# spiraldb/fastlanes

Measured on AMD Instinct MI355X. Metric: billion integers/sec decoded (u32 width-7) + achieved HBM GB/s vs peak, 1-8 GPU, higher is better.
Workload: dtype u32

## Files before the change

__graft_entry__.py:

```python
import os
import subprocess
import sys

ROOT = os.path.dirname(os.path.abspath(__file__))
if ROOT not in sys.path:
    sys.path.insert(0, ROOT)


def build_library():
    jobs = str(min(8, os.cpu_count() or 1))
    subprocess.check_call(["make", "-s", "-j", jobs, "-C", os.path.join(ROOT, "fastlanes_amd", "csrc")])


def build_oracle():
    subprocess.check_call(["make", "-s", "-C", os.path.join(ROOT, "oracle")])


EXAMPLES = ("fused_dict_decode", "iterate_running_max", "fused_for_pack")


def build_examples():
    deps0 = [os.path.join(ROOT, "fastlanes_amd", "csrc", h) for h in ("fl_device.hpp", "fl_kernels.hpp", "fl_tile_map.hpp")]
    outs = {}
    for name in EXAMPLES:
        src = os.path.join(ROOT, "examples", name + ".hip")
        out = os.path.join(ROOT, "examples", "lib" + name + ".so")
        deps = [src] + deps0
        if not os.path.exists(out) or any(os.path.getmtime(d) > os.path.getmtime(out) for d in deps):
            subprocess.check_call(["/opt/rocm/bin/hipcc", "--offload-arch=gfx950", "-O3", "-std=c++17", "-shared", "-fPIC",
                                   "-I", os.path.join(ROOT, "fastlanes_amd", "csrc"), src, "-o", out])
        outs[name] = out
    for name, extra in (("column_decode", []), ("multi_gpu_decode", ["-lpthread"])):
        src = os.path.join(ROOT, "examples", name + ".c")
        exe = os.path.join(ROOT, "examples", name)
        if not os.path.exists(exe) or os.path.getmtime(src) > os.path.getmtime(exe) or \
                os.path.getmtime(os.path.join(ROOT, "include", "fastlanes_amd.h")) > os.path.getmtime(exe):
            subprocess.check_call(["gcc", "-std=c99", "-O2", "-Wall", "-D__HIP_PLATFORM_AMD__", "-I", os.path.join(ROOT, "include"),
                                   "-I", "/opt/rocm/include", src, "-L", os.path.join(ROOT, "fastlanes_amd"), "-lfastlanes_amd",
                                   "-L", "/opt/rocm/lib", "-lamdhip64", "-Wl,-rpath,$ORIGIN/../fastlanes_amd",
                                   "-Wl,-rpath,/opt/rocm/lib"] + extra + ["-o", exe])
        outs[name] = exe
    return outs


def build_checker():
    sys.path.insert(0, os.path.join(ROOT, "tests"))
    from test_gpu_full_check import build_checker as bc
    return bc()


def build():
    build_library()
    build_oracle()
    build_examples()
    build_checker()
    import fastlanes_amd
    lib = fastlanes_amd.load()
    missing = [s for s in fastlanes_amd.exported_symbols() + fastlanes_amd.for_compare_symbols() + fastlanes_amd.select_symbols() +
               fastlanes_amd.aggregate_symbols() + fastlanes_amd.for_compare_range_symbols() + fastlanes_amd.aggregate_by_symbols() + fastlanes_amd.for_compare_columns_symbols() +
               fastlanes_amd.aggregate_columns_symbols() + fastlanes_amd.for_compare_in_symbols() + fastlanes_amd.aggregate_by_columns_symbols() if not hasattr(lib, s)]
    if missing:
        raise RuntimeError(f"libfastlanes_amd.so lacks {missing}")


def smoke():
    import numpy as np
    import torch

    sys.path.insert(0, os.path.join(ROOT, "tests"))
    import fastlanes_amd as fl
    from datagen import values
    from oracle_lib import load_oracle

    assert torch.cuda.is_available(), "smoke() needs cuda:0"
    fl.load()
    oracle = load_oracle()
    dev = torch.device("cuda:0")
    n = 70

    def to_dev(a):
        return torch.from_numpy(a.view(np.uint8)).to(dev).view(getattr(torch, str(a.dtype)))

    def to_np(t, dt):
        return t.view(torch.uint8).cpu().numpy().view(dt)

    pk = values("u32", n * 224, 1)
    got = to_np(fl.BitPacking.unpack(7, to_dev(pk)), np.uint32)
    assert np.array_equal(got, oracle.batch("unpack", "u32", 7, pk)), "unpack u32 W=7 mismatch"
    v = values("u32", n * 1024, 2)
    got = to_np(fl.BitPacking.pack(7, to_dev(v)), np.uint32)
    assert np.array_equal(got, oracle.batch("pack", "u32", 7, v)), "pack u32 W=7 mismatch"
    pk12 = values("u32", n * 384, 3)
    bases = values("u32", n * 32, 4)
    got = to_np(fl.Delta.undelta_pack(12, to_dev(pk12), to_dev(bases)), np.uint32)
    assert np.array_equal(got, oracle.batch("undelta_pack", "u32", 12, pk12, aux=bases)), "undelta_pack mismatch"
    refs = values("u32", n, 5)
    got = to_np(fl.FoR.unfor_pack(7, to_dev(pk), to_dev(refs)), np.uint32)
    assert np.array_equal(got, oracle.batch("unfor_pack", "u32", 7, pk, aux=refs)), "unfor_pack mismatch"
    v64 = values("u64", n * 1024, 6, bits=17)
    d = to_dev(v64)
    assert torch.equal(fl.BitPacking.unpack(17, fl.BitPacking.pack(17, d)).view(torch.int64), d.view(torch.int64))
    v16 = (np.arange(1024) % 8).astype(np.uint16)
    p16 = fl.BitPacking.pack(3, v16)
    assert np.array_equal(p16, oracle.pack("u16", 3, v16))
    assert np.array_equal(fl.BitPacking.unpack(3, p16), v16)
    widths = (1 + np.arange(n) % 32).astype(np.uint8)
    dw = torch.from_numpy(widths).to(dev)
    doff, dtotal = fl.widths_to_offsets("u32", dw)
    off = np.concatenate([[0], np.cumsum(widths.astype(np.int64) * 32)])
    assert int(dtotal.item()) == off[-1] * 4
    col = values("u32", int(off[-1]), 7)
    got = to_np(fl.unpack_widths(dw, doff, to_dev(col)), np.uint32)
    want = np.concatenate([oracle.unpack("u32", int(w), col[off[b]:off[b + 1]]) for b, w in enumerate(widths)])
    assert np.array_equal(got, want), "unpack_widths mismatch"
    brefs = values("u32", n, 8)
    got = to_np(fl.unfor_pack_widths(dw, doff, to_dev(col), to_dev(brefs)), np.uint32)
    want = np.concatenate([oracle.unfor_pack("u32", int(w), col[off[b]:off[b + 1]], brefs[b]) for b, w in enumerate(widths)])
    assert np.array_equal(got, want), "unfor_pack_widths mismatch"
    got = to_np(fl.undelta_pack_widths(dw, doff, to_dev(col), to_dev(bases)), np.uint32)
    want = np.concatenate([oracle.undelta_pack("u32", int(w), col[off[b]:off[b + 1]], bases[b * 32:(b + 1) * 32]) for b, w in enumerate(widths)])
    assert np.array_equal(got, want), "undelta_pack_widths mismatch"
    n8 = 4 * n + 3
    w8 = ((np.arange(n8) * 5) % 9).astype(np.uint8)
    dw8 = torch.from_numpy(w8).to(dev)
    doff8, _ = fl.widths_to_offsets("u8", dw8)
    off8 = np.concatenate([[0], np.cumsum(w8.astype(np.int64) * 128)])
    col8, bases8 = values("u8", int(off8[-1]), 9), values("u8", n8 * 128, 10)
    want = np.concatenate([oracle.undelta_pack("u8", int(w), col8[off8[b]:off8[b + 1]], bases8[b * 128:(b + 1) * 128]) for b, w in enumerate(w8)])
    got = to_np(fl.undelta_pack_widths(dw8, doff8, to_dev(col8), to_dev(bases8)), np.uint8)
    assert np.array_equal(got, want), "undelta_pack_widths u8 mismatch"
# ... 25 lines not shown
```

fastlanes_amd/csrc/fl_capi.hip:

```cpp
#include "../../include/fastlanes_amd.h"
#include "../../include/fastlanes_amd_internal.h"
#include "fl_host.hpp"
#include "fl_kernels.hpp"
#include "fl_misc.hpp"
#include "fl_widths.hpp"
#include "fl_chain.hpp"
#include "fl_stream.hpp"
#include "fl_batch.hpp"
#include "fl_scan.hpp"
#include "fl_consume.hpp"
#include "fl_for_compare.hpp"
#include "fl_for_compare_range.hpp"
#include "fl_for_compare_in.hpp"
#include "fl_aggregate_by_columns.hpp"
#include "fl_select.hpp"
#include "fl_aggregate.hpp"
#include "fl_aggregate_by.hpp"
#include "fl_for_compare_columns.hpp"
#include "fl_aggregate_columns.hpp"
#include "fl_host_tier.hpp"

#include <algorithm>
#include <atomic>
#include <new>
// ... 943 lines not shown
    {                                                                                                     \
        FL_DEVICE_TIER(s, aw, ao, a, ar, bw, bo, b, br, kw, ko, k, kr, mask, res, ef);                    \
        return run_unfor_aggregate_by_columns<T>(ex, {true, 0, aw, ao, ab}, a, ar, ars, {true, 0, bw, bo, bb}, b, br, brs, {true, 0, kw, ko, kb}, k, \
                                                 kr, krs, mask, n, res, ef, s);                           \
    }

FL_DEFINE_AGGREGATE_BY_COLUMNS(uint8_t, u8)
FL_DEFINE_AGGREGATE_BY_COLUMNS(uint16_t, u16)
FL_DEFINE_AGGREGATE_BY_COLUMNS(uint32_t, u32)
FL_DEFINE_AGGREGATE_BY_COLUMNS(uint64_t, u64)

#define FL_DEFINE_FOR_COMPARE_RANGE(T, S)                                                               \
    int fl_##S##_unfor_compare_range(unsigned w, const T* in, const T* r, size_t rs, T lo, T hi, int cb, const uint32_t* mi, size_t n, \
                                     uint32_t* mask, void* s)                                             \
    { FL_DEVICE_TIER(s, in, r, mi, mask); return run_unfor_compare_range<T>({false, w}, in, r, rs, lo, hi, cb, mi, n, mask, nullptr, s); } \
    int fl_##S##_unfor_compare_range_widths(const uint8_t* w, const uint64_t* o, const T* pk, size_t pb, const T* r, size_t rs, T lo, T hi, \
                                            int cb, const uint32_t* mi, size_t n, uint32_t* mask, uint32_t* ef, void* s) \
    { FL_DEVICE_TIER(s, w, o, pk, r, mi, mask, ef); return run_unfor_compare_range<T>({true, 0, w, o, pb}, pk, r, rs, lo, hi, cb, mi, n, mask, ef, s); }

FL_DEFINE_FOR_COMPARE_RANGE(uint8_t, u8)
FL_DEFINE_FOR_COMPARE_RANGE(uint16_t, u16)
FL_DEFINE_FOR_COMPARE_RANGE(uint32_t, u32)
FL_DEFINE_FOR_COMPARE_RANGE(uint64_t, u64)

#define FL_DEFINE_FOR_COMPARE_IN(T, S)                                                                    \
    int fl_##S##_unfor_compare_in(unsigned w, const T* in, const T* r, size_t rs, T lo, uint64_t sb, const uint32_t* sw, int ng, int cb, \
                                  const uint32_t* mi, size_t n, uint32_t* mask, void* s)                  \
    { FL_DEVICE_TIER(s, in, r, sw, mi, mask); return run_unfor_compare_in<T>({false, w}, in, r, rs, lo, sb, sw, ng, cb, mi, n, mask, nullptr, s); } \
    int fl_##S##_unfor_compare_in_widths(const uint8_t* w, const uint64_t* o, const T* pk, size_t pb, const T* r, size_t rs, T lo, uint64_t sb, \
                                         const uint32_t* sw, int ng, int cb, const uint32_t* mi, size_t n, uint32_t* mask, uint32_t* ef, void* s) \
    { FL_DEVICE_TIER(s, w, o, pk, r, sw, mi, mask, ef); return run_unfor_compare_in<T>({true, 0, w, o, pb}, pk, r, rs, lo, sb, sw, ng, cb, mi, n, mask, ef, s); }

FL_DEFINE_FOR_COMPARE_IN(uint8_t, u8)
FL_DEFINE_FOR_COMPARE_IN(uint16_t, u16)
FL_DEFINE_FOR_COMPARE_IN(uint32_t, u32)
FL_DEFINE_FOR_COMPARE_IN(uint64_t, u64)

#define FL_DEFINE_FOR_COMPARE_COLUMNS(T, S)                                                               \
    int fl_##S##_unfor_compare_columns(unsigned wa, const T* a, const T* ar, size_t ars, unsigned wb, const T* b, const T* br, size_t brs, \
                                       int op, int sg, int cb, const uint32_t* mi, size_t n, uint32_t* mask, void* s) \
    {                                                                                                     \
        FL_DEVICE_TIER(s, a, ar, b, br, mi, mask);                                                        \
        return run_unfor_compare_columns<T>({false, wa}, a, ar, ars, {false, wb}, b, br, brs, op, sg, cb, mi, n, mask, nullptr, s); \
    }                                                                                                     \
    int fl_##S##_unfor_compare_columns_widths(const uint8_t* aw, const uint64_t* ao, const T* a, size_t ab, const T* ar, size_t ars, \
                                              const uint8_t* bw, const uint64_t* bo, const T* b, size_t bb, const T* br, size_t brs, \
                                              int op, int sg, int cb, const uint32_t* mi, size_t n, uint32_t* mask, uint32_t* ef, void* s) \
    {                                                                                                     \
        FL_DEVICE_TIER(s, aw, ao, a, ar, bw, bo, b, br, mi, mask, ef);                                    \
        return run_unfor_compare_columns<T>({true, 0, aw, ao, ab}, a, ar, ars, {true, 0, bw, bo, bb}, b, br, brs, op, sg, cb, mi, n, mask, ef, s); \
    }

FL_DEFINE_FOR_COMPARE_COLUMNS(uint8_t, u8)
FL_DEFINE_FOR_COMPARE_COLUMNS(uint16_t, u16)
FL_DEFINE_FOR_COMPARE_COLUMNS(uint32_t, u32)
FL_DEFINE_FOR_COMPARE_COLUMNS(uint64_t, u64)

#define FL_DEFINE_AGGREGATE_COLUMNS(T, S)                                                                 \
    int fl_##S##_unfor_aggregate_columns(int ex, unsigned wa, const T* a, const T* ar, size_t ars, unsigned wb, const T* b, const T* br, \
                                         size_t brs, const uint32_t* mask, size_t n, void* aggs, uint32_t* ef, void* s) \
    {                                                                                                     \
        FL_DEVICE_TIER(s, a, ar, b, br, mask, aggs, ef);                                                  \
        return run_unfor_aggregate_columns<T>(ex, {false, wa}, a, ar, ars, {false, wb}, b, br, brs, mask, n, aggs, ef, s); \
    }                                                                                                     \
    int fl_##S##_unfor_aggregate_columns_widths(int ex, const uint8_t* aw, const uint64_t* ao, const T* a, size_t ab, const T* ar, size_t ars, \
                                                const uint8_t* bw, const uint64_t* bo, const T* b, size_t bb, const T* br, size_t brs, \
                                                const uint32_t* mask, size_t n, void* aggs, uint32_t* ef, void* s) \
    {                                                                                                     \
        FL_DEVICE_TIER(s, aw, ao, a, ar, bw, bo, b, br, mask, aggs, ef);                                  \
        return run_unfor_aggregate_columns<T>(ex, {true, 0, aw, ao, ab}, a, ar, ars, {true, 0, bw, bo, bb}, b, br, brs, mask, n, aggs, ef, s); \
    }

FL_DEFINE_AGGREGATE_COLUMNS(uint8_t, u8)
FL_DEFINE_AGGREGATE_COLUMNS(uint16_t, u16)
FL_DEFINE_AGGREGATE_COLUMNS(uint32_t, u32)
FL_DEFINE_AGGREGATE_COLUMNS(uint64_t, u64)

FL_DEFINE_TYPE(uint8_t, u8)
FL_DEFINE_TYPE(uint16_t, u16)
FL_DEFINE_TYPE(uint32_t, u32)
FL_DEFINE_TYPE(uint64_t, u64)


void fl_internal_set_kernel_policy(int policy)
{
    const KernelPolicy p = policy_fields(policy);
    const bool ok = policy >= 0 && policy < (1 << 30) && p.mode <= 2 && (p.waves == 0 || (p.waves >= 3 && p.waves <= 8)) && p.bpw <= 16
                    && (p.mode == 2 || (p.waves == 0 && p.bpw == 0)) && (p.prefetch == 0 || p.bpw >= 2) && (p.window == 0 || p.window >= 8);
    g_kernel_policy.store(ok ? policy : 0, std::memory_order_relaxed);
    fl::window_override().store(ok ? p.window : 0, std::memory_order_relaxed);
}
int fl_internal_get_kernel_policy(void) { return g_kernel_policy.load(std::memory_order_relaxed); }
uint64_t fl_internal_zero_copy_fallbacks(void) { return g_zero_copy_fallbacks.load(std::memory_order_relaxed); }

int fl_internal_bare_stream(const void* in, size_t in_unit, const void* aux, size_t aux_unit, void* out, size_t out_unit, size_t n_units,
                            int nt_loads, int waves, int window_log2_units, void* stream)
{
    if (n_units == 0) return FL_OK;
    if ((in_unit && !in) || (aux_unit && !aux) || !out) return FL_ERR_NULL;
    if (misaligned(in) || misaligned(aux) || misaligned(out)) return FL_ERR_ALIGN;
    if (in_unit > BARE_MAX_UNIT || out_unit > BARE_MAX_UNIT || aux_unit > 1024 || ((in_unit | out_unit | aux_unit) & 15u)) return FL_ERR_INDEX;
    FL_DEVICE_TIER(stream, in, aux, out);
    BareArgs a{static_cast<const char*>(in), static_cast<const char*>(aux), static_cast<char*>(out), n_units, 0,
               (unsigned)in_unit, (unsigned)aux_unit, (unsigned)out_unit, 63u};
    return hip_status(launch_bare_stream(a, nt_loads != 0, waves, window_log2_units, static_cast<hipStream_t>(stream)));
}

int fl_internal_bare_stream_shape(int op, unsigned type_bits, unsigned width, size_t* in_unit, size_t* aux_unit, size_t* out_unit,
                                  int* nt_loads, int* waves, int* window_log2_units, unsigned* blocks_per_unit)
{
    if (!valid_type_bits(type_bits)) return FL_ERR_INDEX;
    if (op < 0 || op > 3) return FL_ERR_INDEX;
    if (width > (op == 3 ? 2 * type_bits : type_bits)) return FL_ERR_WIDTH;
    if (!in_unit || !aux_unit || !out_unit || !nt_loads || !waves || !window_log2_units || !blocks_per_unit) return FL_ERR_NULL;
    const unsigned k = type_bits == 8 ? 4u : type_bits == 16 ? 2u : 1u;
    const size_t packed = (op == 3 ? 64u * width : 128u * width) * k, unpacked = 128u * type_bits * k;
    *blocks_per_unit = k;
    *in_unit = op == 1 ? unpacked : packed;
    *out_unit = op == 1 ? packed : unpacked;
    *aux_unit = op == 2 ? 128u * k : 0;
    int w = op == 3 ? mixed_waves(type_bits, false) : chosen_waves(type_bits, width, tool_op(op).wave).waves;
    if (w == 0) w = 8;
    *waves = w < 3 ? 3 : w;
    *nt_loads = op == 1 || op == 3 || width >= fl::nt_read_from(type_bits);
    *window_log2_units = window_log2_blocks(tool_op(op).window, type_bits);
    return FL_OK;
}

int fl_internal_selftune_check(int op, unsigned type_bits, unsigned width, const void* in, const void* aux, void* out, size_t n_blocks, void* stream,
                               float* table_ms, float* best_other_ms, int* best_other_policy)
{
    if (!table_ms || !best_other_ms || !best_other_policy) return FL_ERR_NULL;
    if (op < 0 || op > 2 || !valid_type_bits(type_bits)) return FL_ERR_INDEX;
    if (width > type_bits) return FL_ERR_WIDTH;
    hipStream_t s = static_cast<hipStream_t>(stream);
    auto call = [&]() -> int {
        return type_bits == 8 ? selftune_call<uint8_t>(op, width, in, aux, out, n_blocks, stream)
             : type_bits == 16 ? selftune_call<uint16_t>(op, width, in, aux, out, n_blocks, stream)
             : type_bits == 32 ? selftune_call<uint32_t>(op, width, in, aux, out, n_blocks, stream)
                               : selftune_call<uint64_t>(op, width, in, aux, out, n_blocks, stream);
    };
    const int saved = fl_internal_get_kernel_policy();
    int rc = FL_OK;
    auto timed = [&](int policy, float& ms) {
        fl_internal_set_kernel_policy(policy);
        rc = median_ms(s, 1, 3, call, &ms);
    };
    *table_ms = *best_other_ms = 0.f;
    timed(0, *table_ms);
    *best_other_policy = 0;
    const fl::WaveOp wop = tool_op(op).wave;
    const fl::WaveChoice tab = fl::wave_choice(type_bits, width, wop);
    for (int policy : {1, 2 + 256 * 3, 2 + 256 * 4, 2 + 256 * 5, 2 + 256 * 6, 2 + 256 * 8}) {
        if (rc != FL_OK) break;
        if (policy == 1 && (tab.waves == 0 || !fl::cell_column_built(type_bits, width, wop))) continue;
        if (policy != 1 && (policy >> 8) == tab.waves && !tab.two_blocks) continue;
        float ms = 0.f;
        timed(policy, ms);
        if (rc == FL_OK && ms > 0.f && (*best_other_ms == 0.f || ms < *best_other_ms)) { *best_other_ms = ms; *best_other_policy = policy; }
    }
    fl_internal_set_kernel_policy(saved);
    return rc;
}

}
```

fastlanes_amd/csrc/fl_consume.hpp:

```cpp
#pragma once
#include "fl_kernels.hpp"

namespace fl {

constexpr int compare_max_waves(int w) { return w <= 5 ? 8 : w <= 9 ? 3 : 2; }
inline int compare_launch_waves(unsigned type_bits, unsigned w) { return w > 5 ? 0 : type_bits == 8 ? 4 : type_bits == 16 ? 6 : 0; }
constexpr int sums_max_waves(int w) { return (w >= 6 && w <= 12) ? 3 : 8; }

struct ReduceArgs {
    const u32x4* in;
    void* out0;
    void* out1;
    uint64_t n_blocks;
    uint64_t tiles_per_xcd = 0;
    unsigned window_shift = 63;
};

__device__ __forceinline__ bool tile_of_workgroup(const ReduceArgs& a, uint64_t& tile)
{
    const uint64_t n_tiles = (a.n_blocks + BLOCKS_PER_WG - 1) / BLOCKS_PER_WG;
    tile = xcd_tile(blockIdx.x, a.tiles_per_xcd, a.window_shift);
    return tile < n_tiles;
}

// ... 318 lines not shown
{
    using P = InPlaceRows<T, W>;
    constexpr int TB = Elem<T>::BITS;
    auto put = [&](auto J, uint32_t bits) {
        constexpr int j = decltype(J)::value;
        static_assert(j >= 0 && j < TB, "");
        if constexpr (sizeof(T) == 1) *reinterpret_cast<uint16_t*>(lds_blk + j * 16 + c * 2) = (uint16_t)bits;
        else *reinterpret_cast<uint8_t*>(lds_blk + j * 8 + c) = (uint8_t)bits;
    };
    constexpr T FM = W >= TB ? (T) ~(T)0 : (T)(((uint32_t)1 << (W % TB)) - 1u);
    const uint32_t kc = k > FM ? FM : k;
    static_for<(W ? W : 1)>([&](auto WD) {
        constexpr int wd = decltype(WD)::value;
        static_for<2>([&](auto C) {
            constexpr int cl = decltype(C)::value;
            if constexpr (P::any(wd, cl)) {
                constexpr uint32_t M = P::fields(wd, cl), G = P::guards(wd, cl), ONES = P::ones(wd, cl);
                const uint32_t ks = kc * ONES;
                uint32_t t[4];
                for (int i = 0; i < 4; ++i) {
                    if constexpr (IS_EQ) t[i] = G - ((in[wd].x[i] ^ ks) & M);
                    else t[i] = (ks | G) - (in[wd].x[i] & M);
                }
                static_for<TB>([&](auto R) {
                    constexpr int r = decltype(R)::value;
                    static_assert(WaveRowStore<T>::row_at(P::address_row(r)) == r, "address_row inverts row_at");
                    if constexpr (P::member(r, wd, cl))
                        put(std::integral_constant<int, P::address_row(r)>{}, squeeze_bit<T, P::shift(r) + W>(t));
                });
            }
        });
    });
    static_for<TB>([&](auto R) {
        constexpr int r = decltype(R)::value;
        if constexpr (!P::in_place(r))
            put(std::integral_constant<int, P::address_row(r)>{}, row_predicate_bits<T, W, IS_EQ>(unpack_row<T, W, r>(in), (T)kc));
    });
    wave_lds_fence();
    const u32x4 m = *reinterpret_cast<const u32x4*>(lds_blk + c * 16);
    keep[0] = m[0]; keep[1] = m[1]; keep[2] = m[2]; keep[3] = m[3];
    if (IS_EQ && k > FM) keep[0] = keep[1] = keep[2] = keep[3] = 0u;
}

template <typename T, int W, bool IS_EQ>
__global__ __launch_bounds__(WG) __attribute__((amdgpu_waves_per_eu(1, compare_max_waves(W)))) void k_unpack_compare(CompareArgs a)
{
    const uint64_t n_tiles = (a.n_blocks + BLOCKS_PER_WG - 1) / BLOCKS_PER_WG;
    const uint64_t tile = xcd_tile(blockIdx.x, a.tiles_per_xcd, a.window_shift);
    if (tile >= n_tiles) return;
    const unsigned tid = threadIdx.x;
    const uint64_t blk = tile * BLOCKS_PER_WG + (tid >> 3);
    const unsigned c = sizeof(T) >= 4 ? column_of_lane(tid & 7u) : (tid & 7u);
    if (blk >= a.n_blocks) return;
    Cell<T> in[W ? W : 1];
    const u32x4* pk = a.in + blk * (uint64_t)(8 * W) + c;
    static_for<W>([&](auto Wd) { in[decltype(Wd)::value] = load_cell<T, true>(pk + 8 * decltype(Wd)::value); });
    uint32_t keep[4] = {0, 0, 0, 0};
    if constexpr (sizeof(T) >= 4) {
        compare_block_butterfly<T, W, IS_EQ>(in, (T)a.constant, c, keep);
    } else {
        constexpr unsigned MASK_STRIDE = 144;
        __shared__ __attribute__((aligned(16))) char lds[BLOCKS_PER_WG * MASK_STRIDE];
        compare_block_lds<T, W, IS_EQ>(in, (T)a.constant, c, lds + (tid >> 3) * MASK_STRIDE, keep);
    }
    const uint32_t flip = a.invert ? ~0u : 0u;
    const u32x4 out = {keep[0] ^ flip, keep[1] ^ flip, keep[2] ^ flip, keep[3] ^ flip};
    const unsigned wave = __builtin_amdgcn_readfirstlane(tid >> 6);
    const uint64_t wave_first = tile * BLOCKS_PER_WG + wave * 8u;
    const uint64_t left = a.n_blocks - wave_first;
    const __amdgpu_buffer_rsrc_t mask_rs = __builtin_amdgcn_make_buffer_rsrc(
        reinterpret_cast<char*>(a.mask) + wave_first * 128u, 0, (unsigned)(left < 8 ? left : 8) * 128u, 0x00020000);
    __builtin_amdgcn_raw_buffer_store_b128(out, mask_rs, ((tid >> 3) & 7u) * 128u + c * 16u, 0, STORE_AUX);
}

typedef hipError_t (*compare_launch_t)(const CompareArgs&, int waves, hipStream_t);
template <typename T, int W, bool IS_EQ> hipError_t launch_unpack_compare(const CompareArgs& a0, int waves, hipStream_t s)
{
    if (a0.n_blocks == 0) return hipSuccess;
    CompareArgs a = a0;
    const unsigned grid = plan_blocks(a, a.n_blocks, BLOCKS_PER_WG, WIN_UNPACK_COMPARE, Elem<T>::BITS);
    if (!grid) return hipErrorInvalidValue;
    constexpr unsigned STATIC_LDS = sizeof(T) >= 4 ? 0u : BLOCKS_PER_WG * 144u;
    unsigned pad = 0;
    if (waves >= 3 && waves < 8) pad = ((CU_LDS_BYTES / (unsigned)waves) & ~1023u) - STATIC_LDS;
    FL_LAUNCH((k_unpack_compare<T, W, IS_EQ>), dim3(grid), dim3(WG), pad, s, a);
    return hipGetLastError();
}
template <typename T> struct CompareTable { compare_launch_t fn[Elem<T>::BITS + 1]; };
template <typename T, bool IS_EQ, int... Ws>
constexpr CompareTable<T> make_compare_table(std::integer_sequence<int, Ws...>)
{
    return CompareTable<T>{{&launch_unpack_compare<T, Ws, IS_EQ>...}};
}
template <typename T, bool IS_EQ> const CompareTable<T>& compare_table_impl();

typedef hipError_t (*reduce_launch_t)(const ReduceArgs&, hipStream_t);

template <typename T, int W> hipError_t launch_unpack_block_sums(const ReduceArgs& a0, hipStream_t s)
{
    if (a0.n_blocks == 0) return hipSuccess;
    ReduceArgs a = a0;
    const unsigned grid = plan_blocks(a, a.n_blocks, BLOCKS_PER_WG, WIN_UNPACK_BLOCK_SUMS, Elem<T>::BITS);
    if (!grid) return hipErrorInvalidValue;
    FL_LAUNCH((k_unpack_block_sums<T, W>), dim3(grid), dim3(WG), 0, s, a);
    return hipGetLastError();
}
template <typename T> hipError_t launch_block_min_max(const ReduceArgs& a0, hipStream_t s)
{
    if (a0.n_blocks == 0) return hipSuccess;
    ReduceArgs a = a0;
    const unsigned grid = plan_blocks(a, a.n_blocks, BLOCKS_PER_WG, WIN_BLOCK_MIN_MAX, Elem<T>::BITS);
    if (!grid) return hipErrorInvalidValue;
    FL_LAUNCH((k_block_min_max<T>), dim3(grid), dim3(WG), 0, s, a);
    return hipGetLastError();
}

template <typename T> struct ReduceTable { reduce_launch_t fn[Elem<T>::BITS + 1]; };
template <typename T, int... Ws>
constexpr ReduceTable<T> make_sum_table(std::integer_sequence<int, Ws...>)
{
    return ReduceTable<T>{{&launch_unpack_block_sums<T, Ws>...}};
}
template <typename T> const ReduceTable<T>& sum_table_impl();
template <typename T> reduce_launch_t min_max_launcher();

}
```

fastlanes_amd/csrc/fl_dispatch.hpp:

```cpp
#pragma once
#include "fl_dispatch_table.inc"
#include "fl_window_table.inc"

namespace fl {

enum WaveOp { WAVE_UNPACK = 0, WAVE_PACK = 1, WAVE_UNDELTA_PACK = 2, WAVE_UNDELTA = 3, WAVE_DELTA = 4,
              WAVE_UNTRANSPOSE = 5, WAVE_TRANSPOSE = 6, WAVE_UNDELTA_PACK_UNTRANSPOSE = 7, WAVE_TRANSPOSE_DELTA_PACK = 8,
              WAVE_UNFOR_PACK = 9, WAVE_FOR_PACK = 10 };

#define FL_DISPATCH_ROW(NAME, type_bits) \
    ((type_bits) == 64 ? dispatch_table::NAME##_U64 : (type_bits) == 32 ? dispatch_table::NAME##_U32 : \
     (type_bits) == 16 ? dispatch_table::NAME##_U16 : dispatch_table::NAME##_U8)

constexpr int TWO_BLOCKS = 10;
namespace dispatch_table {
template <unsigned N> constexpr bool row_below(const unsigned char (&row)[N], int limit)
{
    for (unsigned i = 0; i < N; ++i)
        if (row[i] >= limit) return false;
    return true;
}
template <unsigned N> constexpr bool two_blocks_row_ok(const unsigned char (&row)[N])
{
    for (unsigned i = 0; i < N; ++i)
        if (row[i] > 8 && (row[i] < TWO_BLOCKS + 4 || row[i] > TWO_BLOCKS + 8)) return false;
    return true;
}
#define FL_CHECK_ROWS(NAME) static_assert(row_below(NAME##_U8, 9) && row_below(NAME##_U16, 9) && row_below(NAME##_U32, 9) && row_below(NAME##_U64, 9), \
                                          "fl_dispatch_table.inc: " #NAME " holds an entry that is not 0 or 3..8 waves per SIMD")
FL_CHECK_ROWS(UNPACK); FL_CHECK_ROWS(PACK); FL_CHECK_ROWS(UNFOR_PACK); FL_CHECK_ROWS(FOR_PACK); FL_CHECK_ROWS(UNDELTA_PACK_UNTRANSPOSE);
FL_CHECK_ROWS(TRANSPOSE_DELTA_PACK); FL_CHECK_ROWS(UNDELTA); FL_CHECK_ROWS(DELTA); FL_CHECK_ROWS(UNTRANSPOSE); FL_CHECK_ROWS(TRANSPOSE);
#undef FL_CHECK_ROWS
static_assert(row_below(UNDELTA_PACK_U8, 9) && row_below(UNDELTA_PACK_U16, 9), "fl_dispatch_table.inc: the two-blocks form exists for u32 / u64 only");
static_assert(two_blocks_row_ok(UNDELTA_PACK_U32) && two_blocks_row_ok(UNDELTA_PACK_U64), "fl_dispatch_table.inc: a two-blocks entry must be 10 + (4..8)");
}
constexpr int unpack_u32_floor(unsigned w, int table) { return (w >= 9 && w < 16 && table > 0 && table < 6) ? 6 : table; }
constexpr int undelta_u64_floor(unsigned w, int table) { return (w >= 8 && w <= 10 && table == 0) ? 6 : table == 3 ? 4 : table; }
constexpr int wave_policy(unsigned type_bits, unsigned w, WaveOp op)
{
    switch (op) {
    case WAVE_UNPACK: return type_bits == 32 ? unpack_u32_floor(w, dispatch_table::UNPACK_U32[w]) : FL_DISPATCH_ROW(UNPACK, type_bits)[w];
    case WAVE_PACK: return FL_DISPATCH_ROW(PACK, type_bits)[w];
    case WAVE_UNFOR_PACK: return FL_DISPATCH_ROW(UNFOR_PACK, type_bits)[w];
    case WAVE_FOR_PACK: return FL_DISPATCH_ROW(FOR_PACK, type_bits)[w];
    case WAVE_UNDELTA_PACK: return type_bits == 64 ? undelta_u64_floor(w, dispatch_table::UNDELTA_PACK_U64[w]) : FL_DISPATCH_ROW(UNDELTA_PACK, type_bits)[w];
    case WAVE_UNDELTA_PACK_UNTRANSPOSE:
        return type_bits == 64 ? undelta_u64_floor(w, dispatch_table::UNDELTA_PACK_UNTRANSPOSE_U64[w]) : FL_DISPATCH_ROW(UNDELTA_PACK_UNTRANSPOSE, type_bits)[w];
    case WAVE_TRANSPOSE_DELTA_PACK: return FL_DISPATCH_ROW(TRANSPOSE_DELTA_PACK, type_bits)[w];
    case WAVE_UNDELTA: return FL_DISPATCH_ROW(UNDELTA, type_bits)[0];
    case WAVE_DELTA: return FL_DISPATCH_ROW(DELTA, type_bits)[0];
    case WAVE_UNTRANSPOSE: return FL_DISPATCH_ROW(UNTRANSPOSE, type_bits)[0];
    default: return FL_DISPATCH_ROW(TRANSPOSE, type_bits)[0];
    }
}

struct WaveChoice {
    int waves;
    bool two_blocks;
};
constexpr WaveChoice wave_choice(unsigned type_bits, unsigned w, WaveOp op)
{
    const int e = wave_policy(type_bits, w, op);
    return e >= TWO_BLOCKS ? WaveChoice{e - TWO_BLOCKS, true} : WaveChoice{e, false};
}

#ifdef FL_ALL_CELL_COLUMN
constexpr bool cell_column_built(unsigned, unsigned, WaveOp) { return true; }
#else
constexpr bool cell_column_built(unsigned type_bits, unsigned w, WaveOp op) { return wave_policy(type_bits, w, op) == 0; }
#endif

constexpr int wave_fallback(unsigned type_bits, bool pack) { return (pack || type_bits <= 16) ? 8 : type_bits == 32 ? 5 : 3; }

inline unsigned uniform_blocks_per_wave(unsigned type_bits, bool  = false, unsigned  = 0, bool  = false)
{
    return type_bits == 8 ? 2u : 1u;
}
inline unsigned mixed_blocks_per_wave(unsigned type_bits, bool pack) { return type_bits == 8 ? (pack ? 2u : 4u) : type_bits == 16 ? 2u : 1u; }
inline unsigned nt_read_from(unsigned type_bits)
{
    static const unsigned div = [] { const char* e = getenv("FL_INTERNAL_NT_FROM_DIV"); const int d = e ? atoi(e) : 0; return d >= 1 && d <= 64 ? (unsigned)d : 0u; }();
    const unsigned d = div ? div : (type_bits >= 32 ? 8u : 2u);
    return (type_bits + d - 1) / d;
}
inline unsigned mixed_prefetch(unsigned type_bits) { return type_bits <= 16 ? 1u : 0u; }
inline int mixed_waves(unsigned type_bits, bool pack) { return (pack || type_bits <= 16) ? 8 : 6; }
inline unsigned batch_blocks_per_wave(unsigned type_bits, bool pack)
{
    return type_bits == 8 ? 4u : type_bits == 16 ? (pack ? 2u : 4u) : (type_bits == 64 && !pack) ? 2u : 1u;
}
inline int batch_waves(unsigned type_bits, bool pack) { return type_bits <= 16 ? 8 : pack ? 6 : type_bits == 64 ? 5 : 8; }

enum WindowOp { WIN_UNPACK = 0, WIN_PACK, WIN_UNDELTA_PACK, WIN_UNDELTA_PACK_UNTRANSPOSE, WIN_TRANSPOSE_DELTA_PACK, WIN_DELTA, WIN_UNDELTA,
                WIN_TRANSPOSE, WIN_UNTRANSPOSE, WIN_UNPACK_COMPARE, WIN_UNPACK_BLOCK_SUMS, WIN_BLOCK_MIN_MAX };
constexpr int window_log2_blocks(WindowOp op, unsigned type_bits)
{
    const int t = type_bits == 8 ? 0 : type_bits == 16 ? 1 : type_bits == 32 ? 2 : 3;
    switch (op) {
    case WIN_UNPACK: return window_table::UNPACK[t];
    case WIN_PACK: return window_table::PACK[t];
    case WIN_UNDELTA_PACK: return window_table::UNDELTA_PACK[t];
    case WIN_UNDELTA_PACK_UNTRANSPOSE: return window_table::UNDELTA_PACK_UNTRANSPOSE[t];
    case WIN_TRANSPOSE_DELTA_PACK: return window_table::TRANSPOSE_DELTA_PACK[t];
    case WIN_DELTA: return window_table::DELTA[t];
    case WIN_UNDELTA: return window_table::UNDELTA[t];
    case WIN_TRANSPOSE: return window_table::TRANSPOSE[t];
    case WIN_UNTRANSPOSE: return window_table::UNTRANSPOSE[t];
    case WIN_UNPACK_COMPARE: return window_table::UNPACK_COMPARE[t];
    case WIN_UNPACK_BLOCK_SUMS: return window_table::UNPACK_BLOCK_SUMS[t];
    default: return window_table::BLOCK_MIN_MAX[t];
    }
}

constexpr unsigned BATCH_MAX_BLOCKS = 1u << 30;

}
```

fastlanes_amd/csrc/fl_kernels.hpp:

```cpp
#pragma once
#include "fl_device.hpp"
#include "fl_dispatch.hpp"
#include "fl_tile_map.hpp"
#include <atomic>

namespace fl {

#ifndef FL_WG
#define FL_WG 256
#endif
constexpr int WG = FL_WG;
constexpr int BLOCKS_PER_WG = WG / 8;

enum UnpackBody { BODY_STORE = 0, BODY_ADD_REF = 1, BODY_UNDELTA = 2,
                  BODY_UNDELTA_UNTRANSPOSE = 3 };
enum PackMode { PACK_PLAIN = 0, PACK_FOR = 1,
                PACK_TRANSPOSE_DELTA = 2 };

struct StreamArgs {
    const u32x4* in;
    u32x4* out;
    const void* aux;
    uint64_t aux_stride;
    uint64_t n_blocks;
    uint64_t tiles_per_xcd = 0;
    unsigned window_shift = 63;
};


inline std::atomic<int>& window_override()
{
    static std::atomic<int> v{0};
    return v;
}
inline int& window_override_this_thread()
{
    static thread_local int v = 0;
    return v;
}
inline bool& constructed_pair_this_thread()
{
    static thread_local bool v = false;
    return v;
}
inline unsigned tile_window_shift(WindowOp op, unsigned type_bits, unsigned tile_blocks)
{
    const int mine = window_override_this_thread();
    const int ov = mine ? mine : window_override().load(std::memory_order_relaxed);
    return window_shift_of(ov ? ov : constructed_pair_this_thread() ? (int)WINDOW_WHOLE : window_log2_blocks(op, type_bits), tile_blocks);
}

template <typename Args>
inline unsigned plan_blocks(Args& a, uint64_t n_blocks, unsigned tile_blocks, WindowOp op, unsigned type_bits, bool rotate = false)
{
    return plan_tiles(a, (n_blocks + tile_blocks - 1) / tile_blocks, tile_window_shift(op, type_bits, tile_blocks) | (rotate ? TILE_MAP_ROTATE : 0u));
}
constexpr unsigned CU_LDS_BYTES = 160 * 1024;
inline unsigned occupancy_lds(int waves, unsigned need = 0)
{
    if (waves < 3) waves = 3;
    const unsigned pad = (CU_LDS_BYTES * (unsigned)WG / ((unsigned)waves * 256u)) & ~1023u;
    return pad > need ? pad : need;
}

#ifndef FL_STORE_AUX
#define FL_STORE_AUX 18
#endif
constexpr int STORE_AUX = FL_STORE_AUX;

template <typename T, int W> struct UnpackPolicy {
    static constexpr int MAXW = 2;
    static constexpr int MAXW_ROWS = 3;
    static constexpr bool NT_LOAD = (2 * W >= Elem<T>::BITS);
};
template <typename T> struct PackPolicy {
    static constexpr int MAXW = sizeof(T) >= 4 ? 1 : 2;
    static constexpr bool NT_LOAD = true;
};

__device__ __forceinline__ bool tile_of_workgroup(const StreamArgs& a, uint64_t& tile)
{
    const uint64_t n_tiles = (a.n_blocks + BLOCKS_PER_WG - 1) / BLOCKS_PER_WG;
    tile = xcd_tile(blockIdx.x, a.tiles_per_xcd, a.window_shift);
    return tile < n_tiles;
}

template <int BLOCK_BYTES> struct TileStore {
    __amdgpu_buffer_rsrc_t rs;
    unsigned vo;
    __device__ __forceinline__ TileStore(u32x4* out, uint64_t tile, uint64_t n_blocks, unsigned tid)
    {
        const uint64_t rem = n_blocks - tile * BLOCKS_PER_WG;
        const unsigned nrec = (unsigned)(rem < BLOCKS_PER_WG ? rem : BLOCKS_PER_WG) * BLOCK_BYTES;
        char* base = reinterpret_cast<char*>(out) + tile * (uint64_t)(BLOCKS_PER_WG * BLOCK_BYTES);
        rs = __builtin_amdgcn_make_buffer_rsrc(base, 0, nrec, 0x00020000);
        vo = (tid >> 3) * BLOCK_BYTES + (tid & 7u) * 16;
    }
    template <typename T> __device__ __forceinline__ void store(unsigned cell_in_block, const Cell<T>& v) const
    {
        __builtin_amdgcn_raw_buffer_store_b128(__builtin_bit_cast(u32x4, v), rs, vo + 16 * cell_in_block, 0, STORE_AUX);
    }
};

template <typename T> struct WaveRowStore {
    static constexpr unsigned BLOCK_BYTES = Elem<T>::CELLS_PER_BLOCK * 16;
    static constexpr int GROUPS = Elem<T>::BITS / 8;
    static constexpr int WAVE_LDS = 8 * 1024;
    __amdgpu_buffer_rsrc_t rs;
    char* lds;
    unsigned lane;
    __device__ __forceinline__ WaveRowStore(u32x4* out, uint64_t first_blk, uint64_t n_blocks, char* wave_lds, unsigned lane_)
    {
        const uint64_t rem = n_blocks - first_blk;
        rs = __builtin_amdgcn_make_buffer_rsrc(reinterpret_cast<char*>(out) + first_blk * BLOCK_BYTES, 0,
                                               (unsigned)(rem < 8 ? rem : 8) * BLOCK_BYTES, 0x00020000);
        lds = wave_lds;
        lane = lane_;
    }
    template <int I> __device__ __forceinline__ void put(const Cell<T>& v) const
    {
        *reinterpret_cast<u32x4*>(lds + (lane >> 3) * 1024 + I * 128 + (lane & 7u) * 16) = __builtin_bit_cast(u32x4, v);
    }
    template <int GROUP> __device__ __forceinline__ void flush() const
    {
        wave_lds_fence();
        static_for<8>([&](auto B) {
            constexpr int b = decltype(B)::value;
            const u32x4 v = *reinterpret_cast<const u32x4*>(lds + b * 1024 + lane * 16);
            __builtin_amdgcn_raw_buffer_store_b128(v, rs, b * BLOCK_BYTES + GROUP * 1024 + lane * 16, 0, STORE_AUX);
        });
        wave_lds_fence();
    }
    __host__ __device__ static constexpr int row_at(int j)
    {
        constexpr int PER_S = Elem<T>::BITS / 8;
        return fl_order((j % PER_S) * (8 / PER_S)) * 8 + j / PER_S;
    }
};

template <typename T, int W, int BODY>
__global__ __launch_bounds__(WG)
__attribute__((amdgpu_waves_per_eu(1, (BODY == BODY_STORE || BODY == BODY_ADD_REF) ? UnpackPolicy<T, W>::MAXW_ROWS
                                                                                    : UnpackPolicy<T, W>::MAXW)))
void k_unpack(StreamArgs a)
{
    constexpr bool NTL = UnpackPolicy<T, W>::NT_LOAD;
// ... 230 lines not shown
```

Baseline: 1422.

## Model LDS allocation granularity to request exact wave occupancy

Adds an occupancy model that accounts for the LDS allocation granule and the per-SIMD wave slots, and uses it to pick the dynamic LDS padding that actually delivers the requested waves per SIMD. The old padding divided CU LDS by the wave count and could land on a different occupancy than intended. It also remaps dispatch-table wave labels to the occupancy actually delivered (e.g. 3→2, 5→4), allows two waves, and adds per-width overrides for u32 and u64 unpack. The risk is that the granule and slot model does not match the real MI355X allocator, which would push kernels to lower or different occupancy than tuned.

```diff
diff --git a/__graft_entry__.py b/__graft_entry__.py
--- a/__graft_entry__.py
+++ b/__graft_entry__.py
@@ -20,7 +20,7 @@
 
 
 def build_examples():
-    deps0 = [os.path.join(ROOT, "fastlanes_amd", "csrc", h) for h in ("fl_device.hpp", "fl_kernels.hpp", "fl_tile_map.hpp")]
+    deps0 = [os.path.join(ROOT, "fastlanes_amd", "csrc", h) for h in ("fl_device.hpp", "fl_kernels.hpp", "fl_tile_map.hpp", "fl_occupancy.hpp")]
     outs = {}
     for name in EXAMPLES:
         src = os.path.join(ROOT, "examples", name + ".hip")
@@ -46,6 +46,8 @@
 def build_checker():
     sys.path.insert(0, os.path.join(ROOT, "tests"))
     from test_gpu_full_check import build_checker as bc
+    from test_gpu_occupancy import build_query
+    build_query()
     return bc()
 
 
diff --git a/fastlanes_amd/csrc/fl_capi.hip b/fastlanes_amd/csrc/fl_capi.hip
--- a/fastlanes_amd/csrc/fl_capi.hip
+++ b/fastlanes_amd/csrc/fl_capi.hip
@@ -1049,13 +1049,17 @@
 FL_DEFINE_TYPE(uint64_t, u64)
 
 
+static void store_kernel_policy(int policy)
+{
+    g_kernel_policy.store(policy, std::memory_order_relaxed);
+    fl::window_override().store(policy_fields(policy).window, std::memory_order_relaxed);
+}
 void fl_internal_set_kernel_policy(int policy)
 {
     const KernelPolicy p = policy_fields(policy);
     const bool ok = policy >= 0 && policy < (1 << 30) && p.mode <= 2 && (p.waves == 0 || (p.waves >= 3 && p.waves <= 8)) && p.bpw <= 16
                     && (p.mode == 2 || (p.waves == 0 && p.bpw == 0)) && (p.prefetch == 0 || p.bpw >= 2) && (p.window == 0 || p.window >= 8);
-    g_kernel_policy.store(ok ? policy : 0, std::memory_order_relaxed);
-    fl::window_override().store(ok ? p.window : 0, std::memory_order_relaxed);
+    store_kernel_policy(ok ? policy : 0);
 }
 int fl_internal_get_kernel_policy(void) { return g_kernel_policy.load(std::memory_order_relaxed); }
 uint64_t fl_internal_zero_copy_fallbacks(void) { return g_zero_copy_fallbacks.load(std::memory_order_relaxed); }
@@ -1088,7 +1092,7 @@
     *aux_unit = op == 2 ? 128u * k : 0;
     int w = op == 3 ? mixed_waves(type_bits, false) : chosen_waves(type_bits, width, tool_op(op).wave).waves;
     if (w == 0) w = 8;
-    *waves = w < 3 ? 3 : w;
+    *waves = w < 2 ? 2 : w;
     *nt_loads = op == 1 || op == 3 || width >= fl::nt_read_from(type_bits);
     *window_log2_units = window_log2_blocks(tool_op(op).window, type_bits);
     return FL_OK;
@@ -1110,7 +1114,7 @@
     const int saved = fl_internal_get_kernel_policy();
     int rc = FL_OK;
     auto timed = [&](int policy, float& ms) {
-        fl_internal_set_kernel_policy(policy);
+        store_kernel_policy(policy);
         rc = median_ms(s, 1, 3, call, &ms);
     };
     *table_ms = *best_other_ms = 0.f;
@@ -1118,7 +1122,7 @@
     *best_other_policy = 0;
     const fl::WaveOp wop = tool_op(op).wave;
     const fl::WaveChoice tab = fl::wave_choice(type_bits, width, wop);
-    for (int policy : {1, 2 + 256 * 3, 2 + 256 * 4, 2 + 256 * 5, 2 + 256 * 6, 2 + 256 * 8}) {
+    for (int policy : {1, 2 + 256 * 2, 2 + 256 * 3, 2 + 256 * 4, 2 + 256 * 5, 2 + 256 * 6, 2 + 256 * 7, 2 + 256 * 8}) {
         if (rc != FL_OK) break;
         if (policy == 1 && (tab.waves == 0 || !fl::cell_column_built(type_bits, width, wop))) continue;
         if (policy != 1 && (policy >> 8) == tab.waves && !tab.two_blocks) continue;
diff --git a/fastlanes_amd/csrc/fl_consume.hpp b/fastlanes_amd/csrc/fl_consume.hpp
--- a/fastlanes_amd/csrc/fl_consume.hpp
+++ b/fastlanes_amd/csrc/fl_consume.hpp
@@ -424,7 +424,7 @@
     if (!grid) return hipErrorInvalidValue;
     constexpr unsigned STATIC_LDS = sizeof(T) >= 4 ? 0u : BLOCKS_PER_WG * 144u;
     unsigned pad = 0;
-    if (waves >= 3 && waves < 8) pad = ((CU_LDS_BYTES / (unsigned)waves) & ~1023u) - STATIC_LDS;
+    if (waves >= 2 && waves < 8) pad = lds_request(waves, STATIC_LDS, 256) - STATIC_LDS;
     FL_LAUNCH((k_unpack_compare<T, W, IS_EQ>), dim3(grid), dim3(WG), pad, s, a);
     return hipGetLastError();
 }
diff --git a/fastlanes_amd/csrc/fl_dispatch.hpp b/fastlanes_amd/csrc/fl_dispatch.hpp
--- a/fastlanes_amd/csrc/fl_dispatch.hpp
+++ b/fastlanes_amd/csrc/fl_dispatch.hpp
@@ -36,7 +36,8 @@
 }
 constexpr int unpack_u32_floor(unsigned w, int table) { return (w >= 9 && w < 16 && table > 0 && table < 6) ? 6 : table; }
 constexpr int undelta_u64_floor(unsigned w, int table) { return (w >= 8 && w <= 10 && table == 0) ? 6 : table == 3 ? 4 : table; }
-constexpr int wave_policy(unsigned type_bits, unsigned w, WaveOp op)
+constexpr int delivered_waves(int label) { return label == 3 ? 2 : label == 5 ? 4 : label; }
+constexpr int wave_label(unsigned type_bits, unsigned w, WaveOp op)
 {
     switch (op) {
     case WAVE_UNPACK: return type_bits == 32 ? unpack_u32_floor(w, dispatch_table::UNPACK_U32[w]) : FL_DISPATCH_ROW(UNPACK, type_bits)[w];
@@ -52,6 +53,19 @@
     case WAVE_UNTRANSPOSE: return FL_DISPATCH_ROW(UNTRANSPOSE, type_bits)[0];
     default: return FL_DISPATCH_ROW(TRANSPOSE, type_bits)[0];
     }
+}
+constexpr int occupancy_post_rule(unsigned type_bits, unsigned w, WaveOp op, int waves)
+{
+    if (op != WAVE_UNPACK) return waves;
+    if (type_bits == 32 && (w == 9 || w == 10)) return 7;
+    if (type_bits == 64 && w >= 13 && w <= 21) return 3;
+    return waves;
+}
+constexpr int wave_policy(unsigned type_bits, unsigned w, WaveOp op)
+{
+    const int e = wave_label(type_bits, w, op);
+    if (e >= TWO_BLOCKS) return TWO_BLOCKS + delivered_waves(e - TWO_BLOCKS);
+    return e == 0 ? 0 : occupancy_post_rule(type_bits, w, op, delivered_waves(e));
 }
 
 struct WaveChoice {
@@ -70,7 +84,7 @@
 constexpr bool cell_column_built(unsigned type_bits, unsigned w, WaveOp op) { return wave_policy(type_bits, w, op) == 0; }
 #endif
 
-constexpr int wave_fallback(unsigned type_bits, bool pack) { return (pack || type_bits <= 16) ? 8 : type_bits == 32 ? 5 : 3; }
+constexpr int wave_fallback(unsigned type_bits, bool pack) { return (pack || type_bits <= 16) ? 8 : type_bits == 32 ? delivered_waves(5) : delivered_waves(3); }
 
 inline unsigned uniform_blocks_per_wave(unsigned type_bits, bool  = false, unsigned  = 0, bool  = false)
 {
@@ -89,7 +103,7 @@
 {
     return type_bits == 8 ? 4u : type_bits == 16 ? (pack ? 2u : 4u) : (type_bits == 64 && !pack) ? 2u : 1u;
 }
-inline int batch_waves(unsigned type_bits, bool pack) { return type_bits <= 16 ? 8 : pack ? 6 : type_bits == 64 ? 5 : 8; }
+inline int batch_waves(unsigned type_bits, bool pack) { return type_bits <= 16 ? 8 : pack ? 6 : type_bits == 64 ? delivered_waves(5) : 8; }
 
 enum WindowOp { WIN_UNPACK = 0, WIN_PACK, WIN_UNDELTA_PACK, WIN_UNDELTA_PACK_UNTRANSPOSE, WIN_TRANSPOSE_DELTA_PACK, WIN_DELTA, WIN_UNDELTA,
                 WIN_TRANSPOSE, WIN_UNTRANSPOSE, WIN_UNPACK_COMPARE, WIN_UNPACK_BLOCK_SUMS, WIN_BLOCK_MIN_MAX };
diff --git a/fastlanes_amd/csrc/fl_kernels.hpp b/fastlanes_amd/csrc/fl_kernels.hpp
--- a/fastlanes_amd/csrc/fl_kernels.hpp
+++ b/fastlanes_amd/csrc/fl_kernels.hpp
@@ -2,6 +2,7 @@
 #include "fl_device.hpp"
 #include "fl_dispatch.hpp"
 #include "fl_tile_map.hpp"
+#include "fl_occupancy.hpp"
 #include <atomic>
 
 namespace fl {
@@ -55,13 +56,7 @@
 {
     return plan_tiles(a, (n_blocks + tile_blocks - 1) / tile_blocks, tile_window_shift(op, type_bits, tile_blocks) | (rotate ? TILE_MAP_ROTATE : 0u));
 }
-constexpr unsigned CU_LDS_BYTES = 160 * 1024;
-inline unsigned occupancy_lds(int waves, unsigned need = 0)
-{
-    if (waves < 3) waves = 3;
-    const unsigned pad = (CU_LDS_BYTES * (unsigned)WG / ((unsigned)waves * 256u)) & ~1023u;
-    return pad > need ? pad : need;
-}
+inline unsigned occupancy_lds(int waves, unsigned need = 0) { return lds_request(waves, need, WG); }
 
 #ifndef FL_STORE_AUX
 #define FL_STORE_AUX 18
diff --git a/fastlanes_amd/csrc/fl_occupancy.hpp b/fastlanes_amd/csrc/fl_occupancy.hpp
--- /dev/null
+++ b/fastlanes_amd/csrc/fl_occupancy.hpp
@@ -0,0 +1,42 @@
+#pragma once
+
+namespace fl {
+
+constexpr unsigned CU_LDS_BYTES = 160 * 1024;
+constexpr unsigned LDS_GRANULE_BYTES = 320 * 4;
+constexpr unsigned CU_LDS_GRANULES = CU_LDS_BYTES / LDS_GRANULE_BYTES;
+constexpr unsigned MAX_DYNAMIC_LDS_BYTES = 64 * 1024;
+constexpr int SIMD_WAVE_SLOTS = 8;
+
+constexpr unsigned lds_granules(unsigned bytes) { return (bytes + LDS_GRANULE_BYTES - 1) / LDS_GRANULE_BYTES; }
+
+constexpr int occupancy_of(unsigned bytes, unsigned wg_threads)
+{
+    const unsigned wg_waves = (wg_threads + 63) / 64;
+    const unsigned slots = 4u * SIMD_WAVE_SLOTS / wg_waves;
+    const unsigned fit = bytes ? CU_LDS_GRANULES / lds_granules(bytes) : slots;
+    return (int)((fit < slots ? fit : slots) * wg_waves / 4u);
+}
+
+constexpr unsigned lds_request(int waves, unsigned need, unsigned wg_threads)
+{
+    if (waves < 2) waves = 2;
+    if (waves > SIMD_WAVE_SLOTS) waves = SIMD_WAVE_SLOTS;
+    if (need > MAX_DYNAMIC_LDS_BYTES) return need;
+    constexpr unsigned TOP = MAX_DYNAMIC_LDS_BYTES / LDS_GRANULE_BYTES;
+    unsigned hi = 0, lo = 0;
+    int best = -1;
+    for (unsigned g = TOP; g >= 1; --g) {
+        const unsigned bytes = (g * LDS_GRANULE_BYTES) & ~1023u;
+        if (bytes < need) break;
+        const int occ = occupancy_of(bytes, wg_threads);
+        if (occ > waves && best >= 0) break;
+        if (occ != best) { best = occ; hi = g; }
+        lo = g;
+        if (occ > waves) break;
+    }
+    if (best < 0) return need;
+    return ((hi == TOP ? lo : hi) * LDS_GRANULE_BYTES) & ~1023u;
+}
+
+}
```

New measurement: 1402. 1.4% lower.
